# JulHoltzDevelopers/WavesAndEigenvalues.jl

Measured on AMD Instinct MI355X. Metric: eigenpairs/sec, higher is better.
Workload: dtype f64

## Files before the change

### wavesandeigenvalues.jl_amd/csrc/debug.hip

```cpp
#include <algorithm>
#include <vector>

#include "solver.h"

namespace {
struct StreamGuard {
    hipStream_t s = nullptr;
    ~StreamGuard() { if (s) (void)hipStreamDestroy(s); }
};
int64_t span(int64_t nv, int64_t stride, int64_t blk) { return nv > 0 ? (nv - 1) * stride + blk : 0; }
void fill_xorshift(std::vector<cplx> &hx) {
    uint64_t s = 0x9E3779B97F4A7C15ull;
    for (auto &v : hx) { s ^= s << 13; s ^= s >> 7; s ^= s << 17; v.x = (double)(s & 0xFFFFF) / 524288.0 - 1.0; v.y = (double)((s >> 20) & 0xFFFFF) / 524288.0 - 1.0; }
}
template <class F> double mean_ms(hipStream_t st, int reps, F &&one) {
    for (int i = 0; i < 3; ++i) one();
    hipEvent_t e0, e1;
    HIP_CHECK(hipEventCreate(&e0));
    HIP_CHECK(hipEventCreate(&e1));
    HIP_CHECK(hipEventRecord(e0, st));
    for (int i = 0; i < reps; ++i) one();
    HIP_CHECK(hipEventRecord(e1, st));
    HIP_CHECK(hipEventSynchronize(e1));
    float ms = 0.f;
// ... 217 lines not shown
            } else if (kind == WAE_GMRES_PAIR) {
                const int64_t onorm = off + (2 * (j + 1) + 3) * N;
                for (int b = 0; b < 2 * nb; ++b) hinv[(size_t)e * 2 * nb + b] = inv2(hpool[onorm + b].x);
            }
        }
        HIP_CHECK(hipSetDevice(device));
        StreamGuard sg;
        HIP_CHECK(hipStreamCreate(&sg.s));
        hipStream_t st = sg.s;
        const size_t nR = (size_t)m * (m + 1) * nb, nrow = (size_t)m * nb;
        DevBuf<cplx> dpool, R, sn, g, vsq, Hraw, rescale, dinv, s_rescale, s_vsq;
        DevBuf<double> cs, sv, sub, hist, relres, bn, s_relres, s_sv;
        DevBuf<int> ints, s_int;
        DevBuf<unsigned char> cmask, ddone, s_cmask;
        const cplx *hc = (const cplx *)cstate;
        dpool.upload(hpool, (size_t)plen, st);
        R.upload(hc, nR, st); sn.upload(hc + nR, nrow, st); g.upload(hc + nR + nrow, nrow + nb, st);
        vsq.upload(hc + nR + 2 * nrow + nb, nrow + 2 * nb, st); Hraw.upload(hc + nR + 3 * nrow + 3 * nb, nR, st);
        cs.upload(dstate, nrow, st); sv.upload(dstate + nrow, nrow + 2 * nb, st); sub.upload(dstate + 2 * nrow + 2 * nb, nrow, st);
        hist.upload(dstate + 3 * nrow + 2 * nb, (size_t)histcap * nb, st);
        bn.upload(bnorm, (size_t)nb, st);
        ddone.upload(hdone.data(), hdone.size(), st);
        dinv.upload(hinv.data(), hinv.size(), st);
        relres.alloc(nb); rescale.alloc(nb); ints.alloc(nint); cmask.alloc(nch);
        HIP_CHECK(hipMemsetAsync(ints.p, 0, (size_t)nint * sizeof(int), st));
        HIP_CHECK(hipMemsetAsync(relres.p, 0, (size_t)nb * sizeof(double), st));
        HIP_CHECK(hipMemsetAsync(rescale.p, 0, (size_t)nb * sizeof(cplx), st));
        HIP_CHECK(hipMemsetAsync(cmask.p, 0, (size_t)nch, st));
        s_relres.alloc((size_t)nev * nb); s_int.alloc((size_t)nev * nint); s_cmask.alloc((size_t)nev * nch); s_rescale.alloc((size_t)nev * nb);
        s_sv.alloc((size_t)nev * 2 * nb); s_vsq.alloc((size_t)nev * 2 * nb);
        HIP_CHECK(hipMemsetAsync(s_sv.p, 0, (size_t)nev * 2 * nb * sizeof(double), st));
        HIP_CHECK(hipMemsetAsync(s_vsq.p, 0, (size_t)nev * 2 * nb * sizeof(cplx), st));
        GmresDev S;
        S.nb = nb; S.m = m; S.histcap = histcap;
        S.R = R.p; S.cs = cs.p; S.sn = sn.p; S.g = g.p; S.sv = sv.p; S.vsq = vsq.p;
        S.conv = ints.p; S.steps = S.conv + nb; S.iters = S.steps + nb; S.histlen = S.iters + nb; S.stalled = S.histlen + nb; S.status = S.stalled + nb;
        S.relres = relres.p; S.bnorm = bn.p; S.hist = hist.p; S.rescale = rescale.p; S.cmask = cmask.p;
        S.Hraw = Hraw.p; S.sub = sub.p;
        auto d2d = [&](void *dst, const void *src, size_t bytes) { HIP_CHECK(hipMemcpyAsync(dst, src, bytes, hipMemcpyDeviceToDevice, st)); };
        for (int e = 0, ii = 0; e < nev; ++e) {
            const int64_t kind = ev[4 * e], j = ev[4 * e + 1], off = ev[4 * e + 3];
            const int use_mask = ev[4 * e + 2] ? 1 : 0;
            const double tol = evd[2 * e], lim = evd[2 * e + 1];
            cplx *a = dpool.p + off;
            int row0 = -1, rows = 0;
            if (kind == WAE_GMRES_INIT) {
                launch_gmres_init(S, a, ddone.p + (size_t)ii * nb, use_mask, st);
                ++ii;
                row0 = 0; rows = 1;
            } else if (kind == WAE_GMRES_STEP) {
                d2d(vsq.p + (size_t)(j + 1) * nb, dinv.p + (size_t)e * 2 * nb, (size_t)nb * sizeof(cplx));
                launch_gmres_step(S, a, (int)j, tol, lim, use_mask, a + (j + 2) * N, n, st);
                row0 = (int)j + 1; rows = 1;
            } else if (kind == WAE_GMRES_PAIR) {
                cplx *c1 = a, *c2 = c1 + (j + 1) * N, *gram = c2 + (j + 1) * N, *norms = gram + 3 * N, *W1 = norms + 2 * N, *W2 = W1 + blk,
                     *alpha = W2 + blk, *c2m = alpha + N, *hd2 = c2m + (j + 1) * N;
                launch_gmres_pair_coef(S, (int)j, c1, c2, gram, alpha, c2m, hd2, st);
                d2d(vsq.p + (size_t)(j + 1) * nb, dinv.p + (size_t)e * 2 * nb, (size_t)2 * nb * sizeof(cplx));
                launch_gmres_step(S, c1, (int)j, tol, 1e300, use_mask, W1, n, st, norms);
                launch_gmres_step(S, hd2, (int)j + 1, tol, lim, use_mask, W2, n, st, norms + N);
                row0 = (int)j + 1; rows = 2;
            } else {
                launch_gmres_solve_y(S, (int)j, a, st);
            }
            d2d(s_relres.p + (size_t)e * nb, relres.p, (size_t)nb * sizeof(double));
            d2d(s_int.p + (size_t)e * nint, ints.p, (size_t)nint * sizeof(int));
            d2d(s_cmask.p + (size_t)e * nch, cmask.p, (size_t)nch);
            d2d(s_rescale.p + (size_t)e * nb, rescale.p, (size_t)nb * sizeof(cplx));
            if (rows) {
                d2d(s_sv.p + (size_t)e * 2 * nb, sv.p + (size_t)row0 * nb, (size_t)rows * nb * sizeof(double));
                d2d(s_vsq.p + (size_t)e * 2 * nb, vsq.p + (size_t)row0 * nb, (size_t)rows * nb * sizeof(cplx));
            }
        }
        auto back = [&](void *dst, const void *src, size_t bytes) { HIP_CHECK(hipMemcpyAsync(dst, src, bytes, hipMemcpyDeviceToHost, st)); };
        cplx *oc = (cplx *)cstate;
        back(pool, dpool.p, (size_t)plen * sizeof(cplx));
        back(oc, R.p, nR * sizeof(cplx)); back(oc + nR, sn.p, nrow * sizeof(cplx)); back(oc + nR + nrow, g.p, (nrow + nb) * sizeof(cplx));
        back(oc + nR + 2 * nrow + nb, vsq.p, (nrow + 2 * nb) * sizeof(cplx)); back(oc + nR + 3 * nrow + 3 * nb, Hraw.p, nR * sizeof(cplx));
        back(dstate, cs.p, nrow * sizeof(double)); back(dstate + nrow, sv.p, (nrow + 2 * nb) * sizeof(double));
        back(dstate + 2 * nrow + 2 * nb, sub.p, nrow * sizeof(double)); back(dstate + 3 * nrow + 2 * nb, hist.p, (size_t)histcap * nb * sizeof(double));
        back(snap_relres, s_relres.p, (size_t)nev * nb * sizeof(double)); back(snap_int, s_int.p, (size_t)nev * nint * sizeof(int));
        back(snap_cmask, s_cmask.p, (size_t)nev * nch); back(snap_rescale, s_rescale.p, (size_t)nev * nb * sizeof(cplx));
        back(snap_sv, s_sv.p, (size_t)nev * 2 * nb * sizeof(double)); back(snap_vsq, s_vsq.p, (size_t)nev * 2 * nb * sizeof(cplx));
// ... 286 lines not shown
```

### wavesandeigenvalues.jl_amd/csrc/gmres.hip

```cpp
#include <cmath>

#include "solver.h"

void upload_pc(wae_family *h, const std::vector<std::vector<zc>> &pcs) {
    const int nsys = (int)pcs.size();
    const int nl = (int)h->ops.size();
    const size_t per_level = (size_t)nsys * h->nplanes;
    std::vector<cplx> tab(per_level * (nl + 2));
    for (int l = 0; l <= nl + 1; ++l) {
        if (l >= nl && h->n_penalty == 0) break;
        const std::vector<int> &sp = l < nl ? h->slot_plane[l] : (l == nl ? h->pen_slot : h->pen_row_slot);
        for (int s = 0; s < nsys; ++s) slot_coeffs(h, sp, pcs[s], &tab[l * per_level + (size_t)s * h->nplanes]);
    }
    h->pc_stride_level = per_level;
    h->pcdev.upload(tab.data(), tab.size(), h->stream);
    HIP_CHECK(hipStreamSynchronize(h->stream));
}
const cplx *pc_level(const wae_family *h, int l) { return h->pcdev.p + (size_t)l * h->pc_stride_level; }

void dense_setup(wae_family *h, const Batch &bt) {
    const int L = (int)h->ops.size() - 1;
    if (h->nc <= 0) return;
    HIP_CHECK(hipMemsetAsync(h->dstatus.p, 0, sizeof(int), h->stream));
    launch_dense_assemble(h->dense_planes.p, h->nplanes, (int)h->nc, pc_level(h, L), bt.nsys, bt.op, h->Ainv.p, h->stream);
// ... 245 lines not shown
                itot += iters[b];
                if (bnorm[b] > 0.0) {
                    if (!(relres[b] <= tol)) ++nun;
                    rmax = std::max(rmax, relres[b]);
                }
                if (stalled[b] && !(relres[b] <= tol)) info->levels |= 1 << 16;
            }
            info->iters_max = std::max(info->iters_max, imax);
            info->iters_total += itot;
            info->n_unconverged += nun;
            info->relres_max = std::max(info->relres_max, rmax);
            info->levels = (info->levels & (1 << 16)) | (int)h->ops.size();
        }
        if (nan_seen) throw WaeError(WAE_ERR_NAN, "NaN in GMRES");
        return total_it;
    }

    int run_device(wae_solve_info *info) {
        const GmresEnv &env = gmres_env();
        const double lim = env.lazy_limit;
        const bool use_mask = have_x0 || (env.mask0 && nb >= 8);
        const int nch = (nb + 7) / 8;
        const int histcap = maxit + m + 8;
        h->gs_R.reserve((size_t)m * (m + 1) * nb); h->gs_sn.reserve((size_t)m * nb); h->gs_g.reserve((size_t)(m + 1) * nb); h->gs_rescale.reserve((size_t)nb);
        h->gs_cs.reserve((size_t)m * nb); h->gs_sv.reserve((size_t)(m + 2) * nb); h->gs_relres.reserve((size_t)nb); h->gs_bnorm.reserve((size_t)nb);
        h->gs_hist.reserve((size_t)histcap * nb); h->gs_int.reserve((size_t)5 * nb + 4); h->gs_done.reserve((size_t)nb);
        h->cmask.reserve(nch); h->vsq.reserve((size_t)(m + 2) * nb);
        GmresDev S;
        S.nb = nb; S.m = m; S.histcap = histcap;
        S.R = h->gs_R.p; S.cs = h->gs_cs.p; S.sn = h->gs_sn.p; S.g = h->gs_g.p; S.sv = h->gs_sv.p; S.vsq = h->vsq.p;
        S.conv = h->gs_int.p; S.steps = S.conv + nb; S.iters = S.steps + nb; S.histlen = S.iters + nb; S.stalled = S.histlen + nb; S.status = S.stalled + nb;
        S.relres = h->gs_relres.p; S.bnorm = h->gs_bnorm.p; S.hist = h->gs_hist.p; S.rescale = h->gs_rescale.p; S.cmask = h->cmask.p;
        const int pair_min = env.pair_min;
        const bool pair_on = pair_min >= 0 && lim >= 1e50 && nb >= 8 && h->ops.size() > 1;
        h->gs_Hraw.reserve((size_t)m * (m + 1) * nb); h->gs_pair.reserve(((size_t)4 * (m + 3) + 8) * nb); h->gs_sub.reserve((size_t)m * nb);
        S.Hraw = h->gs_Hraw.p; S.sub = h->gs_sub.p;
        cplx *const pr_c1 = h->gs_pair.p, *const pr_c2 = pr_c1 + (size_t)(m + 3) * nb, *const pr_c2m = pr_c2 + (size_t)(m + 3) * nb,
                   *const pr_hd2 = pr_c2m + (size_t)(m + 3) * nb, *const pr_gram = pr_hd2 + (size_t)(m + 3) * nb, *const pr_alpha = pr_gram + (size_t)3 * nb,
                   *const pr_norm = pr_alpha + nb;
        HIP_CHECK(hipMemsetAsync(h->gs_int.p, 0, ((size_t)5 * nb + 4) * sizeof(int), st));
        cplx *const zb = start();
        std::vector<double> bn(bnorm);
        for (double &v : bn) if (!(v > 0.0)) v = 1.0;
        HIP_CHECK(hipMemcpyAsync(h->gs_bnorm.p, bn.data(), nb * sizeof(double), hipMemcpyHostToDevice, st));
        HIP_CHECK(hipStreamSynchronize(st));
        std::vector<int> hostint((size_t)5 * nb + 4);
        bool first = !have_x0;
// ... 8 lines not shown
            if (cycle_start([](int) {}) || total_it >= maxit || nan_seen) break;
            launch_scale_inv(z0, h->hdev.p, h->V.p, n, nb, st);
            HIP_CHECK(hipMemcpyAsync(h->gs_done.p, done.data(), nb, hipMemcpyHostToDevice, st));
            launch_gmres_init(S, h->hdev.p, h->gs_done.p, use_mask ? 1 : 0, st);
            HIP_CHECK(hipStreamSynchronize(st));
            const unsigned char *mk = (use_mask && nb >= 8) ? h->cmask.p : nullptr;
            int j = 0;
            int status[4] = {0, 0, 0, 0};
            for (int b = 0; b < nb; ++b) status[0] += done[b] ? 0 : 1;
            int since_sync = 0;
            for (; j < m && total_it < maxit;) {
                const cplx *vj = h->V.p + (size_t)j * vec;
                const int nvj = j + 1;
                const bool fuse0 = h->ops.size() > 1;
                if (pair_on && j >= pair_min && j + 2 <= m && total_it + 2 <= maxit && status[0] > nb / 4) {
                    cplx *w1 = h->V.p + (size_t)nvj * vec, *w2 = w1 + vec;
                    launch_spmv(A, pc, bt.cps, vj, h->W.p, h->lx[0].p, pre_weight(h), nb, MODE_AX_J0, st, mk);
                    vcycle(h, bt, 0, h->W.p, mk, true, w1);
                    launch_spmv(A, pc, bt.cps, w1, h->W.p, h->lx[0].p, pre_weight(h), nb, MODE_AX_J0, st, mk);
                    vcycle(h, bt, 0, h->W.p, mk, true, w2);
                    launch_dots2_scaled(h->V.p, vec, nvj, w1, w2, n, nb, h->partial.p, pr_c1, pr_c2, pr_gram, h->vsq.p, st, mk);
                    launch_gmres_pair_coef(S, j, pr_c1, pr_c2, pr_gram, pr_alpha, pr_c2m, pr_hd2, st);
                    launch_axpy2_norm(h->V.p, vec, nvj, pr_c1, pr_c2m, pr_alpha, w1, w2, n, nb, h->partial.p, pr_norm, h->vsq.p + (size_t)nvj * nb, st, mk);
                    launch_gmres_step(S, pr_c1, j, tol, 1e300, use_mask ? 1 : 0, w1, n, st, pr_norm);
                    launch_gmres_step(S, pr_hd2, j + 1, tol, lim, use_mask ? 1 : 0, w2, n, st, pr_norm + nb);
                    j += 2;
                    total_it += 2;
                    since_sync += 2;
                } else {
                    launch_spmv(A, pc, bt.cps, vj, h->W.p, fuse0 ? h->lx[0].p : nullptr, fuse0 ? pre_weight(h) : 0.0, nb, fuse0 ? MODE_AX_J0 : MODE_AX, st, mk);
                    cplx *w = vcycle(h, bt, 0, h->W.p, mk, fuse0);
                    launch_dots_scaled(h->V.p, vec, nvj, w, n, nb, h->partial.p, h->hdev.p, h->vsq.p, st, mk);
                    launch_axpy_neg_norm(h->V.p, vec, nvj, h->hdev.p, h->V.p + (size_t)nvj * vec, n, nb, h->partial.p, h->hdev.p + (size_t)nvj * nb, st, mk,
                                         w, h->vsq.p + (size_t)nvj * nb);
                    launch_gmres_step(S, h->hdev.p, j, tol, lim, use_mask ? 1 : 0, h->V.p + (size_t)nvj * vec, n, st);
                    ++j;
                    ++total_it;
                    ++since_sync;
                }
                if (since_sync >= ((have_x0 && j <= 4) ? 1 : env.sync) || j == m || total_it >= maxit || status[0] <= nb / 4) {
                    since_sync = 0;
                    HIP_CHECK(hipMemcpyAsync(status, S.status, 3 * sizeof(int), hipMemcpyDeviceToHost, st));
                    HIP_CHECK(hipStreamSynchronize(st));
                    if (status[1]) nan_seen = true;
                    if (status[0] == 0 || nan_seen) break;
                }
            }
            if (j > 0) {
// ... 434 lines not shown
```

### wavesandeigenvalues.jl_amd/csrc/vec.hip

```cpp
#include <type_traits>

#include "block_reduce.h"
#include "kernel_helpers.h"

__global__ void fill_zero_kernel(cplx *X, size_t count) {
    for (size_t e = (size_t)blockIdx.x * 256 + threadIdx.x; e < count; e += (size_t)gridDim.x * 256) X[e] = cplx{0.0, 0.0};
}
void launch_fill_zero(cplx *X, size_t count, hipStream_t st) {
    if (!count) return;
    hipLaunchKernelGGL(fill_zero_kernel, dim3(grid_for(count)), dim3(256), 0, st, X, count);
    HIP_CHECK(hipGetLastError());
}
void launch_copy(const cplx *X, cplx *Y, size_t count, hipStream_t st) {
    if (!count) return;
    HIP_CHECK(hipMemcpyAsync(Y, X, count * sizeof(cplx), hipMemcpyDeviceToDevice, st));
}
__global__ void add_kernel(const cplx *__restrict__ X, cplx *__restrict__ Y, size_t count) {
    for (size_t e = (size_t)blockIdx.x * 256 + threadIdx.x; e < count; e += (size_t)gridDim.x * 256) {
        cplx a = X[e], b = Y[e];
        Y[e] = cplx{a.x + b.x, a.y + b.y};
    }
}
void launch_add(const cplx *X, cplx *Y, size_t count, hipStream_t st) {
    if (!count) return;
// ... 742 lines not shown

__global__ __launch_bounds__(256) void gmres_init_kernel(GmresDev S, const cplx *__restrict__ beta, const unsigned char *__restrict__ done, int use_mask) {
    __shared__ int act[256];
    const int b = threadIdx.x;
    int a = 0;
    if (b < S.nb) {
        S.g[b] = cplx{beta[b].x, 0.0};
        S.sv[b] = 1.0;
        S.vsq[b] = cplx{1.0, 0.0};
        S.conv[b] = done[b] ? 1 : 0;
        S.steps[b] = 0;
        a = done[b] ? 0 : 1;
    }
    act[b] = a;
    __syncthreads();
    if (b < (S.nb + 7) / 8) {
        int any = 0;
        for (int k = 0; k < 8; ++k) any |= act[b * 8 + k];
        S.cmask[b] = use_mask ? (unsigned char)any : (unsigned char)1;
    }
    if (b == 0) {
        int n = 0;
        for (int k = 0; k < S.nb; ++k) n += act[k];
        S.status[0] = n; S.status[1] = 0; S.status[2] = 0;
    }
}

__global__ __launch_bounds__(256) void gmres_step_kernel(GmresDev S, const cplx *__restrict__ hd, int j, double tol, double lim, int use_mask,
                                                         const cplx *__restrict__ rn) {
    __shared__ int act[256];
    const int b = threadIdx.x;
    const int nb = S.nb, m = S.m;
    int a = 0;
    if (b < nb) {
        const int nvj = j + 1;
        const double sj = S.sv[(size_t)j * nb + b];
        const double r = rn ? rn[b].x : hd[(size_t)nvj * nb + b].x;
        if (S.Hraw) {
            cplx *Hr = S.Hraw + (size_t)j * (m + 1) * nb;
            for (int i = 0; i <= j; ++i) Hr[(size_t)i * nb + b] = hd[(size_t)i * nb + b];
        }
        double svn = r > 0.0 ? 1.0 / r : 0.0;
        const bool resc = svn > lim || (svn > 0.0 && svn < 1.0 / lim);
        S.rescale[b] = resc ? cplx{r, 0.0} : cplx{0.0, 0.0};
        if (S.sub) S.sub[(size_t)j * nb + b] = resc ? r : 1.0;
        if (resc) {
            S.vsq[(size_t)nvj * nb + b] = cplx{svn > 0.0 ? 1.0 : 0.0, 0.0};
            svn = svn > 0.0 ? 1.0 : 0.0;
            atomicOr(&S.status[2], 1);
        }
        S.sv[(size_t)nvj * nb + b] = svn;
        if (!S.conv[b]) {
            cplx *Hc = S.R + (size_t)j * (m + 1) * nb;
            for (int i = 0; i <= j; ++i) {
                const double si = S.sv[(size_t)i * nb + b];
                const double f = si > 0.0 ? sj / si : 0.0;
                const cplx c = hd[(size_t)i * nb + b];
                Hc[(size_t)i * nb + b] = cplx{c.x * f, c.y * f};
            }
            Hc[(size_t)(j + 1) * nb + b] = cplx{sj * r, 0.0};
            for (int i = 0; i < j; ++i) {
                const cplx aa = Hc[(size_t)i * nb + b], bb = Hc[(size_t)(i + 1) * nb + b];
                const double c = S.cs[(size_t)i * nb + b];
                const cplx sn = S.sn[(size_t)i * nb + b];
                const cplx sb = cmul(sn, bb), ca = cmul(cconj(sn), aa);
                Hc[(size_t)i * nb + b] = cplx{c * aa.x + sb.x, c * aa.y + sb.y};
                Hc[(size_t)(i + 1) * nb + b] = cplx{-ca.x + c * bb.x, -ca.y + c * bb.y};
            }
            const cplx av = Hc[(size_t)j * nb + b];
            const double bv = Hc[(size_t)(j + 1) * nb + b].x;
            const double aabs = hypot(av.x, av.y);
            const double t = sqrt(aabs * aabs + bv * bv);
            if (!(t > 0.0) || isnan(t)) {
                S.conv[b] = 1;
                if (isnan(t)) atomicOr(&S.status[1], 1);
            } else {
                double c;
                cplx sn;
                if (aabs == 0.0) { c = 0.0; sn = cplx{1.0, 0.0}; }
                else { c = aabs / t; const double q = bv / t; sn = cplx{av.x / aabs * q, av.y / aabs * q}; }
                S.cs[(size_t)j * nb + b] = c;
                S.sn[(size_t)j * nb + b] = sn;
                Hc[(size_t)j * nb + b] = cplx{c * av.x + sn.x * bv, c * av.y + sn.y * bv};
                Hc[(size_t)(j + 1) * nb + b] = cplx{0.0, 0.0};
                const cplx gj = S.g[(size_t)j * nb + b];
                const cplx gn = cmul(cconj(sn), gj);
                S.g[(size_t)(j + 1) * nb + b] = cplx{-gn.x, -gn.y};
                S.g[(size_t)j * nb + b] = cplx{c * gj.x, c * gj.y};
                S.steps[b] = j + 1;
                S.iters[b] += 1;
                const double rr = hypot(gn.x, gn.y) / S.bnorm[b];
                S.relres[b] = rr;
                if (isnan(rr)) atomicOr(&S.status[1], 1);
                const int hs = S.histlen[b];
                if (hs < S.histcap) { S.hist[(size_t)hs * nb + b] = rr; S.histlen[b] = hs + 1; }
                const int hn = hs + 1;
                if (rr <= 0.7 * tol) S.conv[b] = 1;
                else if (hn > 60 && hs < S.histcap && rr > 0.9 * S.hist[(size_t)(hn - 31) * nb + b]) { S.conv[b] = 1; S.stalled[b] = 1; }
                else a = 1;
            }
        }
    }
    act[b] = a;
    __syncthreads();
    if (b < (nb + 7) / 8 && use_mask) {
        int any = 0;
        for (int k = 0; k < 8; ++k) any |= act[b * 8 + k];
        S.cmask[b] = (unsigned char)any;
    }
    if (b == 0) {
        int n = 0;
        for (int k = 0; k < nb; ++k) n += act[k];
        S.status[0] = n;
    }
}

__global__ __launch_bounds__(256) void gmres_solve_y_kernel(GmresDev S, int ju, cplx *__restrict__ out) {
    const int b = threadIdx.x;
    const int nb = S.nb, m = S.m;
    if (b >= nb) return;
    const int k = S.steps[b];
    for (int i = k; i < ju; ++i) out[(size_t)i * nb + b] = cplx{0.0, 0.0};
    for (int i = k - 1; i >= 0; --i) {
        cplx sacc = S.g[(size_t)i * nb + b];
        for (int q = i + 1; q < k; ++q) {
            const cplx hq = S.R[((size_t)q * (m + 1) + i) * nb + b];
            const cplx yq = out[(size_t)q * nb + b];
            sacc.x -= hq.x * yq.x - hq.y * yq.y;
            sacc.y -= hq.x * yq.y + hq.y * yq.x;
        }
        const cplx dg = S.R[((size_t)i * (m + 1) + i) * nb + b];
        out[(size_t)i * nb + b] = (dg.x != 0.0 || dg.y != 0.0) ? cdiv(sacc, dg) : cplx{0.0, 0.0};
    }
    for (int i = 0; i < k; ++i) {
        const double f = S.sv[(size_t)i * nb + b];
        cplx y = out[(size_t)i * nb + b];
        out[(size_t)i * nb + b] = cplx{f * y.x, f * y.y};
    }
}

__global__ __launch_bounds__(256) void gmres_rescale_kernel(cplx *__restrict__ V, const cplx *__restrict__ factor, const int *__restrict__ status, size_t total, int nb) {
    if (!status[2]) return;
    for (size_t e = (size_t)blockIdx.x * 256 + threadIdx.x; e < total; e += (size_t)gridDim.x * 256) {
        const double f = factor[e % nb].x;
        if (f > 0.0) { const cplx x = V[e]; V[e] = cplx{x.x / f, x.y / f}; }
    }
}
__global__ void gmres_clear_rescale_kernel(int *status) { status[2] = 0; }

void launch_gmres_init(const GmresDev &S, const cplx *beta, const unsigned char *done, int use_mask, hipStream_t st) {
    hipLaunchKernelGGL(gmres_init_kernel, dim3(1), dim3(256), 0, st, S, beta, done, use_mask);
    HIP_CHECK(hipGetLastError());
}
__global__ __launch_bounds__(256) void gmres_pair_coef_kernel(GmresDev S, int j, const cplx *__restrict__ c1, const cplx *__restrict__ c2,
                                                              const cplx *__restrict__ gram, cplx *__restrict__ alpha, cplx *__restrict__ c2m,
                                                              cplx *__restrict__ hd2) {
    const int b = threadIdx.x;
    const int nb = S.nb, m = S.m;
    if (b >= nb) return;
    double uu = gram[b].x;
    cplx u12 = gram[(size_t)nb + b];
    for (int i = 0; i <= j; ++i) {
        const double q = S.vsq[(size_t)i * nb + b].x;
        const double w = q > 0.0 ? 1.0 / q : 0.0;
        const cplx a = c1[(size_t)i * nb + b], c = c2[(size_t)i * nb + b];
        uu -= (a.x * a.x + a.y * a.y) * w;
        u12.x -= (a.x * c.x + a.y * c.y) * w;
        u12.y -= (a.x * c.y - a.y * c.x) * w;
    }
    cplx al = {0.0, 0.0};
    if (uu > 0.0 && uu > 1e-28 * gram[b].x) al = cplx{u12.x / uu, u12.y / uu};
// ... 1 lines not shown
    cplx *Hj = S.Hraw + (size_t)j * (m + 1) * nb;
    for (int i = 0; i <= j; ++i) {
        const cplx a = c1[(size_t)i * nb + b], c = c2[(size_t)i * nb + b];
        Hj[(size_t)i * nb + b] = a;
        c2m[(size_t)i * nb + b] = cplx{c.x - (al.x * a.x - al.y * a.y), c.y - (al.x * a.y + al.y * a.x)};
    }
    S.sub[(size_t)j * nb + b] = 1.0;
    for (int i = 0; i <= j + 1; ++i) {
        cplx t = i <= j ? c2[(size_t)i * nb + b] : al;
        for (int k = i; k <= j; ++k) {
            const cplx hk = S.Hraw[((size_t)k * (m + 1) + i) * nb + b], ck = c1[(size_t)k * nb + b];
            t.x -= hk.x * ck.x - hk.y * ck.y;
            t.y -= hk.x * ck.y + hk.y * ck.x;
        }
        if (i >= 1) {
            const double sb = S.sub[(size_t)(i - 1) * nb + b];
            const cplx ck = c1[(size_t)(i - 1) * nb + b];
            t.x -= sb * ck.x;
            t.y -= sb * ck.y;
        }
        hd2[(size_t)i * nb + b] = t;
    }
}
void launch_gmres_pair_coef(const GmresDev &S, int j, const cplx *c1, const cplx *c2, const cplx *gram, cplx *alpha, cplx *c2m, cplx *hd2, hipStream_t st) {
    hipLaunchKernelGGL(gmres_pair_coef_kernel, dim3(1), dim3(256), 0, st, S, j, c1, c2, gram, alpha, c2m, hd2);
    HIP_CHECK(hipGetLastError());
}
void launch_gmres_step(const GmresDev &S, const cplx *hd, int j, double tol, double lim, int use_mask, cplx *Vnew, int64_t n, hipStream_t st,
                       const cplx *rn) {
    hipLaunchKernelGGL(gmres_step_kernel, dim3(1), dim3(256), 0, st, S, hd, j, tol, lim, use_mask, rn);
    hipLaunchKernelGGL(gmres_rescale_kernel, dim3(512), dim3(256), 0, st, Vnew, S.rescale, S.status, (size_t)n * S.nb, S.nb);
    hipLaunchKernelGGL(gmres_clear_rescale_kernel, dim3(1), dim3(1), 0, st, S.status);
    HIP_CHECK(hipGetLastError());
}
void launch_gmres_solve_y(const GmresDev &S, int ju, cplx *out, hipStream_t st) {
    hipLaunchKernelGGL(gmres_solve_y_kernel, dim3(1), dim3(256), 0, st, S, ju, out);
    HIP_CHECK(hipGetLastError());
}

__global__ __launch_bounds__(256) void triad_kernel(double2 *__restrict__ a, const double2 *__restrict__ b, const double2 *__restrict__ c, double s, size_t n2) {
    for (size_t e = (size_t)blockIdx.x * 256 + threadIdx.x; e < n2; e += (size_t)gridDim.x * 256) {
        double2 x = b[e], y = c[e];
        a[e] = double2{x.x + s * y.x, x.y + s * y.y};
    }
}
void launch_triad(double *a, const double *b, const double *c, double s_, int64_t n, hipStream_t st, unsigned grid_cap) {
    size_t n2 = (size_t)n / 2;
    hipLaunchKernelGGL(triad_kernel, dim3(grid_for(n2, grid_cap)), dim3(256), 0, st, (double2 *)a, (const double2 *)b, (const double2 *)c, s_, n2);
    HIP_CHECK(hipGetLastError());
}

constexpr int PTG_MAXW = 3072;
template <int TMAX>
__global__ __launch_bounds__(256) void pt_gemm_batch_kernel(const cplx *__restrict__ V, size_t stride, int k, const cplx *__restrict__ G, int T, int t0,
                                                            int tn, cplx *__restrict__ U, int64_t d, int nb, int accumulate) {
    extern __shared__ cplx ptg_w[];
    const int tid = threadIdx.x;
    for (int e = tid; e < k * tn * nb; e += 256) {
        const int b = e % nb, it = e / nb, t = it % tn, i = it / tn;
// ... 104 lines not shown
```

### wavesandeigenvalues.jl_amd/csrc/wae_internal.h

```cpp
#pragma once
#include <hip/hip_runtime.h>
#include <algorithm>
#include <cmath>
#include <complex>
#include <cstdint>
#include <cstdio>
#include <cstring>
#include <stdexcept>
#include <string>
#include <vector>

#include "../../include/waehip.h"

typedef std::complex<double> zc;
typedef double2 cplx;

struct WaeError : std::runtime_error {
    int code;
    WaeError(int c, const std::string &m) : std::runtime_error(m), code(c) {}
};
void wae_set_error(const std::string &m);
int wae_internal_device(const wae_family *h);
hipStream_t wae_internal_stream(const wae_family *h);

// ... 291 lines not shown
    cplx *R;
    double *cs;
    cplx *sn;
    cplx *g;
    double *sv;
    cplx *vsq;
    int *conv, *steps, *iters, *histlen, *stalled;
    double *relres, *bnorm;
    double *hist;
    cplx *rescale;
    int *status;
    unsigned char *cmask;
    cplx *Hraw;
    double *sub;
};
void launch_gmres_init(const GmresDev &S, const cplx *beta, const unsigned char *done, int use_mask, hipStream_t s);
void launch_gmres_step(const GmresDev &S, const cplx *hd, int j, double tol, double lim, int use_mask, cplx *Vnew, int64_t n, hipStream_t s,
                       const cplx *rn = nullptr);
void launch_dots2_scaled(const cplx *V, size_t stride, int nv, const cplx *W1, const cplx *W2, int64_t n, int nb, cplx *partial, cplx *out1,
                         cplx *out2, cplx *gram_out, const cplx *scale, hipStream_t s, const unsigned char *cmask = nullptr);
void launch_axpy2_norm(const cplx *V, size_t stride, int nv, const cplx *c1, const cplx *c2m, const cplx *alpha, cplx *W1, cplx *W2, int64_t n, int nb,
                       cplx *partial, cplx *norms, cplx *inv_out, hipStream_t s, const unsigned char *cmask = nullptr);
void launch_gmres_pair_coef(const GmresDev &S, int j, const cplx *c1, const cplx *c2, const cplx *gram, cplx *alpha, cplx *c2m, cplx *hd2, hipStream_t s);
void launch_gmres_solve_y(const GmresDev &S, int ju, cplx *out, hipStream_t s);
void launch_forced_rhs(const int *rows, const cplx *M, int64_t nr, int nsrc, const cplx *G, cplx *B, int nb, hipStream_t s);
void launch_forced_observe(const int64_t *ptr, const int *idx, const cplx *val, int nobs, const cplx *X, int nb, cplx *H, int64_t j0, hipStream_t s);
void launch_triad(double *a, const double *b, const double *c, double s, int64_t n, hipStream_t st, unsigned grid_cap = 8192);
```

Measured before the change: 4.433.

## Fuse paired GMRES steps into one LDS-staged kernel and parallelize small solves

Paired Arnoldi columns now go through a single step kernel that applies both Givens updates in one launch. The Hessenberg column and Givens coefficients are staged in shared memory, the rescale kernel handles both vectors together, and the clear-rescale launch is dropped. The pair-coefficient and triangular-solve kernels gain LDS-backed multi-block variants that spread the work across more workgroups instead of one block. This targets launch overhead and serial global-memory latency in these small single-block kernels. In exchange it adds LDS-size fallbacks, a larger rescale buffer and new status-slot semantics that must stay consistent.

```diff
diff --git a/wavesandeigenvalues.jl_amd/csrc/debug.hip b/wavesandeigenvalues.jl_amd/csrc/debug.hip
--- a/wavesandeigenvalues.jl_amd/csrc/debug.hip
+++ b/wavesandeigenvalues.jl_amd/csrc/debug.hip
@@ -263,10 +263,10 @@
         bn.upload(bnorm, (size_t)nb, st);
         ddone.upload(hdone.data(), hdone.size(), st);
         dinv.upload(hinv.data(), hinv.size(), st);
-        relres.alloc(nb); rescale.alloc(nb); ints.alloc(nint); cmask.alloc(nch);
+        relres.alloc(nb); rescale.alloc((size_t)2 * nb); ints.alloc(nint); cmask.alloc(nch);
         HIP_CHECK(hipMemsetAsync(ints.p, 0, (size_t)nint * sizeof(int), st));
         HIP_CHECK(hipMemsetAsync(relres.p, 0, (size_t)nb * sizeof(double), st));
-        HIP_CHECK(hipMemsetAsync(rescale.p, 0, (size_t)nb * sizeof(cplx), st));
+        HIP_CHECK(hipMemsetAsync(rescale.p, 0, (size_t)2 * nb * sizeof(cplx), st));
         HIP_CHECK(hipMemsetAsync(cmask.p, 0, (size_t)nch, st));
         s_relres.alloc((size_t)nev * nb); s_int.alloc((size_t)nev * nint); s_cmask.alloc((size_t)nev * nch); s_rescale.alloc((size_t)nev * nb);
         s_sv.alloc((size_t)nev * 2 * nb); s_vsq.alloc((size_t)nev * 2 * nb);
@@ -298,8 +298,7 @@
                      *alpha = W2 + blk, *c2m = alpha + N, *hd2 = c2m + (j + 1) * N;
                 launch_gmres_pair_coef(S, (int)j, c1, c2, gram, alpha, c2m, hd2, st);
                 d2d(vsq.p + (size_t)(j + 1) * nb, dinv.p + (size_t)e * 2 * nb, (size_t)2 * nb * sizeof(cplx));
-                launch_gmres_step(S, c1, (int)j, tol, 1e300, use_mask, W1, n, st, norms);
-                launch_gmres_step(S, hd2, (int)j + 1, tol, lim, use_mask, W2, n, st, norms + N);
+                launch_gmres_pair_step(S, c1, hd2, (int)j, tol, 1e300, lim, use_mask, W1, W2, n, st, norms);
                 row0 = (int)j + 1; rows = 2;
             } else {
                 launch_gmres_solve_y(S, (int)j, a, st);
diff --git a/wavesandeigenvalues.jl_amd/csrc/gmres.hip b/wavesandeigenvalues.jl_amd/csrc/gmres.hip
--- a/wavesandeigenvalues.jl_amd/csrc/gmres.hip
+++ b/wavesandeigenvalues.jl_amd/csrc/gmres.hip
@@ -291,7 +291,7 @@
         const bool use_mask = have_x0 || (env.mask0 && nb >= 8);
         const int nch = (nb + 7) / 8;
         const int histcap = maxit + m + 8;
-        h->gs_R.reserve((size_t)m * (m + 1) * nb); h->gs_sn.reserve((size_t)m * nb); h->gs_g.reserve((size_t)(m + 1) * nb); h->gs_rescale.reserve((size_t)nb);
+        h->gs_R.reserve((size_t)m * (m + 1) * nb); h->gs_sn.reserve((size_t)m * nb); h->gs_g.reserve((size_t)(m + 1) * nb); h->gs_rescale.reserve((size_t)2 * nb);
         h->gs_cs.reserve((size_t)m * nb); h->gs_sv.reserve((size_t)(m + 2) * nb); h->gs_relres.reserve((size_t)nb); h->gs_bnorm.reserve((size_t)nb);
         h->gs_hist.reserve((size_t)histcap * nb); h->gs_int.reserve((size_t)5 * nb + 4); h->gs_done.reserve((size_t)nb);
         h->cmask.reserve(nch); h->vsq.reserve((size_t)(m + 2) * nb);
@@ -346,8 +346,7 @@
                     launch_dots2_scaled(h->V.p, vec, nvj, w1, w2, n, nb, h->partial.p, pr_c1, pr_c2, pr_gram, h->vsq.p, st, mk);
                     launch_gmres_pair_coef(S, j, pr_c1, pr_c2, pr_gram, pr_alpha, pr_c2m, pr_hd2, st);
                     launch_axpy2_norm(h->V.p, vec, nvj, pr_c1, pr_c2m, pr_alpha, w1, w2, n, nb, h->partial.p, pr_norm, h->vsq.p + (size_t)nvj * nb, st, mk);
-                    launch_gmres_step(S, pr_c1, j, tol, 1e300, use_mask ? 1 : 0, w1, n, st, pr_norm);
-                    launch_gmres_step(S, pr_hd2, j + 1, tol, lim, use_mask ? 1 : 0, w2, n, st, pr_norm + nb);
+                    launch_gmres_pair_step(S, pr_c1, pr_hd2, j, tol, 1e300, lim, use_mask ? 1 : 0, w1, w2, n, st, pr_norm);
                     j += 2;
                     total_it += 2;
                     since_sync += 2;
diff --git a/wavesandeigenvalues.jl_amd/csrc/vec.hip b/wavesandeigenvalues.jl_amd/csrc/vec.hip
--- a/wavesandeigenvalues.jl_amd/csrc/vec.hip
+++ b/wavesandeigenvalues.jl_amd/csrc/vec.hip
@@ -788,103 +788,188 @@
     if (b == 0) {
         int n = 0;
         for (int k = 0; k < S.nb; ++k) n += act[k];
-        S.status[0] = n; S.status[1] = 0; S.status[2] = 0;
-    }
-}
-
-__global__ __launch_bounds__(256) void gmres_step_kernel(GmresDev S, const cplx *__restrict__ hd, int j, double tol, double lim, int use_mask,
-                                                         const cplx *__restrict__ rn) {
+        S.status[0] = n; S.status[1] = 0; S.status[2] = 0; S.status[3] = 0;
+    }
+}
+
+constexpr size_t GMRES_LDS_BUDGET = 144 * 1024;
+static void gmres_lds_opt_in(const void *kernel) { HIP_CHECK(hipFuncSetAttribute(kernel, hipFuncAttributeMaxDynamicSharedMemorySize, (int)GMRES_LDS_BUDGET)); }
+
+struct GmresColumn { int conv, iters, hs; double bnorm; cplx g; };
+
+__device__ __forceinline__ void gmres_stage_column(const GmresDev &S, const cplx *__restrict__ hd, int j, const double *sjl, cplx *Hc) {
+    const int nb = S.nb, total = (j + 1) * nb;
+    cplx *Hr = S.Hraw ? S.Hraw + (size_t)j * (S.m + 1) * nb : nullptr;
+    for (int e0 = threadIdx.x; e0 < total; e0 += 4 * 256) {
+        cplx c[4];
+        double si[4];
+#pragma unroll
+        for (int u = 0; u < 4; ++u) {
+            const int e = e0 + u * 256;
+            c[u] = cplx{0.0, 0.0}; si[u] = 0.0;
+            if (e < total) { c[u] = hd[e]; si[u] = S.sv[e]; }
+        }
+#pragma unroll
+        for (int u = 0; u < 4; ++u) {
+            const int e = e0 + u * 256;
+            if (e < total) {
+                const int i = e / nb, b = e - i * nb;
+                const double sj = sjl[b], s = i == j ? sj : si[u];
+                const double f = s > 0.0 ? sj / s : 0.0;
+                if (Hr) Hr[e] = c[u];
+                Hc[e] = cplx{c[u].x * f, c[u].y * f};
+            }
+        }
+    }
+}
+
+__device__ __forceinline__ int gmres_step_column(const GmresDev &S, const cplx *__restrict__ hd, int j, double tol, double lim, const cplx *__restrict__ rn,
+                                                 int b, bool staged, bool keep, cplx *Hc, double *csl, cplx *snl, double sj, cplx *resc_out,
+                                                 GmresColumn &col, int &resc_any, double &svn_out) {
+    const int nb = S.nb, m = S.m, nvj = j + 1;
+    const double r = rn ? rn[b].x : hd[(size_t)nvj * nb + b].x;
+    if (!staged && S.Hraw) {
+        cplx *Hr = S.Hraw + (size_t)j * (m + 1) * nb;
+        for (int i = 0; i <= j; ++i) Hr[(size_t)i * nb + b] = hd[(size_t)i * nb + b];
+    }
+    double svn = r > 0.0 ? 1.0 / r : 0.0;
+    const bool resc = svn > lim || (svn > 0.0 && svn < 1.0 / lim);
+    resc_out[b] = resc ? cplx{r, 0.0} : cplx{0.0, 0.0};
+    if (S.sub) S.sub[(size_t)j * nb + b] = resc ? r : 1.0;
+    if (resc) {
+        S.vsq[(size_t)nvj * nb + b] = cplx{svn > 0.0 ? 1.0 : 0.0, 0.0};
+        svn = svn > 0.0 ? 1.0 : 0.0;
+        resc_any = 1;
+    }
+    S.sv[(size_t)nvj * nb + b] = svn;
+    svn_out = svn;
+    if (col.conv) return 0;
+    if (!staged) {
+        for (int i = 0; i <= j; ++i) {
+            const double si = S.sv[(size_t)i * nb + b];
+            const double f = si > 0.0 ? sj / si : 0.0;
+            const cplx c = hd[(size_t)i * nb + b];
+            Hc[(size_t)i * nb + b] = cplx{c.x * f, c.y * f};
+        }
+    }
+    const double bv = sj * r;
+    cplx aa = Hc[b];
+    for (int i = 0; i < j; ++i) {
+        const cplx bb = Hc[(size_t)(i + 1) * nb + b];
+        const double c = csl[(size_t)i * nb + b];
+        const cplx sn = snl[(size_t)i * nb + b];
+        const cplx sb = cmul(sn, bb), ca = cmul(cconj(sn), aa);
+        Hc[(size_t)i * nb + b] = cplx{c * aa.x + sb.x, c * aa.y + sb.y};
+        aa = cplx{-ca.x + c * bb.x, -ca.y + c * bb.y};
+    }
+    const cplx av = aa;
+    const double aabs = hypot(av.x, av.y);
+    const double t = sqrt(aabs * aabs + bv * bv);
+    int a = 0;
+    if (!(t > 0.0) || isnan(t)) {
+        Hc[(size_t)j * nb + b] = av;
+        Hc[(size_t)(j + 1) * nb + b] = cplx{bv, 0.0};
+        col.conv = 1;
+        S.conv[b] = 1;
+        if (isnan(t)) atomicOr(&S.status[1], 1);
+    } else {
+        double c;
+        cplx sn;
+        if (aabs == 0.0) { c = 0.0; sn = cplx{1.0, 0.0}; }
+        else { c = aabs / t; const double q = bv / t; sn = cplx{av.x / aabs * q, av.y / aabs * q}; }
+        S.cs[(size_t)j * nb + b] = c;
+        S.sn[(size_t)j * nb + b] = sn;
+        if (keep) { csl[(size_t)j * nb + b] = c; snl[(size_t)j * nb + b] = sn; }
+        Hc[(size_t)j * nb + b] = cplx{c * av.x + sn.x * bv, c * av.y + sn.y * bv};
+        Hc[(size_t)(j + 1) * nb + b] = cplx{0.0, 0.0};
+        const cplx gj = col.g;
+        const cplx gn = cmul(cconj(sn), gj);
+        col.g = cplx{-gn.x, -gn.y};
+        S.g[(size_t)(j + 1) * nb + b] = col.g;
+        S.g[(size_t)j * nb + b] = cplx{c * gj.x, c * gj.y};
+        S.steps[b] = j + 1;
+        col.iters += 1;
+        S.iters[b] = col.iters;
+        const double rr = hypot(gn.x, gn.y) / col.bnorm;
+        S.relres[b] = rr;
+        if (isnan(rr)) atomicOr(&S.status[1], 1);
+        const int hs = col.hs;
+        if (hs < S.histcap) { S.hist[(size_t)hs * nb + b] = rr; col.hs = hs + 1; S.histlen[b] = hs + 1; }
+        const int hn = hs + 1;
+        if (rr <= 0.7 * tol) { col.conv = 1; S.conv[b] = 1; }
+        else if (hn > 60 && hs < S.histcap && rr > 0.9 * S.hist[(size_t)(hn - 31) * nb + b]) { col.conv = 1; S.conv[b] = 1; S.stalled[b] = 1; }
+        else a = 1;
+    }
+    if (staged) {
+        cplx *Rc = S.R + (size_t)j * (m + 1) * nb;
+        for (int i = 0; i <= j + 1; ++i) Rc[(size_t)i * nb + b] = Hc[(size_t)i * nb + b];
+    }
+    return a;
+}
+
+__global__ __launch_bounds__(256) void gmres_step_kernel(GmresDev S, const cplx *__restrict__ hd1, const cplx *__restrict__ hd2, int j, double tol,
+                                                         double lim1, double lim2, int use_mask, const cplx *__restrict__ rn, int staged) {
+    extern __shared__ cplx step_lds[];
     __shared__ int act[256];
+    __shared__ double sjl[256];
     const int b = threadIdx.x;
     const int nb = S.nb, m = S.m;
-    int a = 0;
+    const int jmax = hd2 ? j + 1 : j;
+    cplx *Hl = step_lds, *snl = Hl + (size_t)(jmax + 2) * nb;
+    double *csl = (double *)(snl + (size_t)jmax * nb);
+    GmresColumn col = {1, 0, 0, 1.0, cplx{0.0, 0.0}};
     if (b < nb) {
-        const int nvj = j + 1;
-        const double sj = S.sv[(size_t)j * nb + b];
-        const double r = rn ? rn[b].x : hd[(size_t)nvj * nb + b].x;
-        if (S.Hraw) {
-            cplx *Hr = S.Hraw + (size_t)j * (m + 1) * nb;
-            for (int i = 0; i <= j; ++i) Hr[(size_t)i * nb + b] = hd[(size_t)i * nb + b];
-        }
-        double svn = r > 0.0 ? 1.0 / r : 0.0;
-        const bool resc = svn > lim || (svn > 0.0 && svn < 1.0 / lim);
-        S.rescale[b] = resc ? cplx{r, 0.0} : cplx{0.0, 0.0};
-        if (S.sub) S.sub[(size_t)j * nb + b] = resc ? r : 1.0;
-        if (resc) {
-            S.vsq[(size_t)nvj * nb + b] = cplx{svn > 0.0 ? 1.0 : 0.0, 0.0};
-            svn = svn > 0.0 ? 1.0 : 0.0;
-            atomicOr(&S.status[2], 1);
-        }
-        S.sv[(size_t)nvj * nb + b] = svn;
-        if (!S.conv[b]) {
-            cplx *Hc = S.R + (size_t)j * (m + 1) * nb;
-            for (int i = 0; i <= j; ++i) {
-                const double si = S.sv[(size_t)i * nb + b];
-                const double f = si > 0.0 ? sj / si : 0.0;
-                const cplx c = hd[(size_t)i * nb + b];
-                Hc[(size_t)i * nb + b] = cplx{c.x * f, c.y * f};
-            }
-            Hc[(size_t)(j + 1) * nb + b] = cplx{sj * r, 0.0};
-            for (int i = 0; i < j; ++i) {
-                const cplx aa = Hc[(size_t)i * nb + b], bb = Hc[(size_t)(i + 1) * nb + b];
-                const double c = S.cs[(size_t)i * nb + b];
-                const cplx sn = S.sn[(size_t)i * nb + b];
-                const cplx sb = cmul(sn, bb), ca = cmul(cconj(sn), aa);
-                Hc[(size_t)i * nb + b] = cplx{c * aa.x + sb.x, c * aa.y + sb.y};
-                Hc[(size_t)(i + 1) * nb + b] = cplx{-ca.x + c * bb.x, -ca.y + c * bb.y};
-            }
-            const cplx av = Hc[(size_t)j * nb + b];
-            const double bv = Hc[(size_t)(j + 1) * nb + b].x;
-            const double aabs = hypot(av.x, av.y);
-            const double t = sqrt(aabs * aabs + bv * bv);
-            if (!(t > 0.0) || isnan(t)) {
-                S.conv[b] = 1;
-                if (isnan(t)) atomicOr(&S.status[1], 1);
-            } else {
-                double c;
-                cplx sn;
-                if (aabs == 0.0) { c = 0.0; sn = cplx{1.0, 0.0}; }
-                else { c = aabs / t; const double q = bv / t; sn = cplx{av.x / aabs * q, av.y / aabs * q}; }
-                S.cs[(size_t)j * nb + b] = c;
-                S.sn[(size_t)j * nb + b] = sn;
-                Hc[(size_t)j * nb + b] = cplx{c * av.x + sn.x * bv, c * av.y + sn.y * bv};
-                Hc[(size_t)(j + 1) * nb + b] = cplx{0.0, 0.0};
-                const cplx gj = S.g[(size_t)j * nb + b];
-                const cplx gn = cmul(cconj(sn), gj);
-                S.g[(size_t)(j + 1) * nb + b] = cplx{-gn.x, -gn.y};
-                S.g[(size_t)j * nb + b] = cplx{c * gj.x, c * gj.y};
-                S.steps[b] = j + 1;
-                S.iters[b] += 1;
-                const double rr = hypot(gn.x, gn.y) / S.bnorm[b];
-                S.relres[b] = rr;
-                if (isnan(rr)) atomicOr(&S.status[1], 1);
-                const int hs = S.histlen[b];
-                if (hs < S.histcap) { S.hist[(size_t)hs * nb + b] = rr; S.histlen[b] = hs + 1; }
-                const int hn = hs + 1;
-                if (rr <= 0.7 * tol) S.conv[b] = 1;
-                else if (hn > 60 && hs < S.histcap && rr > 0.9 * S.hist[(size_t)(hn - 31) * nb + b]) { S.conv[b] = 1; S.stalled[b] = 1; }
-                else a = 1;
-            }
-        }
+        col = GmresColumn{S.conv[b], S.iters[b], S.histlen[b], S.bnorm[b], S.g[(size_t)j * nb + b]};
+        sjl[b] = S.sv[(size_t)j * nb + b];
+    }
+    if (staged) {
+        const int total = j * nb;
+        for (int e0 = b; e0 < total; e0 += 4 * 256) {
+            cplx s[4];
+            double c[4];
+#pragma unroll
+            for (int u = 0; u < 4; ++u) {
+                const int e = e0 + u * 256;
+                s[u] = cplx{0.0, 0.0}; c[u] = 0.0;
+                if (e < total) { s[u] = S.sn[e]; c[u] = S.cs[e]; }
+            }
+#pragma unroll
+            for (int u = 0; u < 4; ++u) {
+                const int e = e0 + u * 256;
+                if (e < total) { snl[e] = s[u]; csl[e] = c[u]; }
+            }
+        }
+    }
+    __syncthreads();
+    if (staged) gmres_stage_column(S, hd1, j, sjl, Hl);
+    __syncthreads();
+    int a = 0, resc_any = 0;
+    double svn = 0.0;
+    if (b < nb)
+        a = gmres_step_column(S, hd1, j, tol, lim1, rn, b, staged, staged && hd2, staged ? Hl : S.R + (size_t)j * (m + 1) * nb, staged ? csl : S.cs,
+                              staged ? snl : S.sn, sjl[b], hd2 ? S.rescale + nb : S.rescale, col, resc_any, svn);
+    if (hd2) {
+        if (b < nb) sjl[b] = svn;
+        __syncthreads();
+        if (staged) gmres_stage_column(S, hd2, j + 1, sjl, Hl);
+        __syncthreads();
+        if (b < nb)
+            a = gmres_step_column(S, hd2, j + 1, tol, lim2, rn + nb, b, staged, false, staged ? Hl : S.R + (size_t)(j + 1) * (m + 1) * nb,
+                                  staged ? csl : S.cs, staged ? snl : S.sn, svn, S.rescale, col, resc_any, svn);
     }
     act[b] = a;
-    __syncthreads();
+    const int nact = __syncthreads_count(a);
+    const int anyr = __syncthreads_or(resc_any);
     if (b < (nb + 7) / 8 && use_mask) {
         int any = 0;
         for (int k = 0; k < 8; ++k) any |= act[b * 8 + k];
         S.cmask[b] = (unsigned char)any;
     }
-    if (b == 0) {
-        int n = 0;
-        for (int k = 0; k < nb; ++k) n += act[k];
-        S.status[0] = n;
-    }
-}
-
-__global__ __launch_bounds__(256) void gmres_solve_y_kernel(GmresDev S, int ju, cplx *__restrict__ out) {
-    const int b = threadIdx.x;
+    if (b == 0) { S.status[0] = nact; S.status[3] = anyr ? 1 : 0; }
+}
+
+__device__ __forceinline__ void gmres_solve_y_column(const GmresDev &S, int ju, cplx *__restrict__ out, int b) {
     const int nb = S.nb, m = S.m;
-    if (b >= nb) return;
     const int k = S.steps[b];
     for (int i = k; i < ju; ++i) out[(size_t)i * nb + b] = cplx{0.0, 0.0};
     for (int i = k - 1; i >= 0; --i) {
@@ -904,15 +989,85 @@
         out[(size_t)i * nb + b] = cplx{f * y.x, f * y.y};
     }
 }
-
-__global__ __launch_bounds__(256) void gmres_rescale_kernel(cplx *__restrict__ V, const cplx *__restrict__ factor, const int *__restrict__ status, size_t total, int nb) {
-    if (!status[2]) return;
+__global__ __launch_bounds__(256) void gmres_solve_y_kernel(GmresDev S, int ju, cplx *__restrict__ out) {
+    if ((int)threadIdx.x < S.nb) gmres_solve_y_column(S, ju, out, threadIdx.x);
+}
+__global__ __launch_bounds__(256) void gmres_solve_y_lds_kernel(GmresDev S, int ju, cplx *__restrict__ out, int cpw) {
+    extern __shared__ cplx solve_lds[];
+    __shared__ int ks[256];
+    const int tid = threadIdx.x;
+    const int nb = S.nb, m = S.m;
+    const int b0 = blockIdx.x * cpw;
+    const int nc = min(cpw, nb - b0);
+    const int T = ju * (ju + 1) / 2;
+    cplx *tri = solve_lds, *gl = tri + (size_t)T * cpw, *yl = gl + (size_t)ju * cpw;
+    if (tid < nc) ks[tid] = S.steps[b0 + tid];
+    __syncthreads();
+    const int total = ju * ju * nc;
+    for (int e0 = tid; e0 < total; e0 += 8 * 256) {
+        cplx v[8];
+        int at[8];
+#pragma unroll
+        for (int u = 0; u < 8; ++u) {
+            const int e = e0 + u * 256;
+            at[u] = -1;
+            v[u] = cplx{0.0, 0.0};
+            if (e < total) {
+                const int c = e % nc, r = e / nc, q = r / ju, i = r - q * ju;
+                if (i <= q && q < ks[c]) {
+                    at[u] = (q * (q + 1) / 2 + i) * cpw + c;
+                    v[u] = S.R[((size_t)q * (m + 1) + i) * nb + b0 + c];
+                }
+            }
+        }
+#pragma unroll
+        for (int u = 0; u < 8; ++u)
+            if (at[u] >= 0) tri[at[u]] = v[u];
+    }
+    for (int e = tid; e < ju * nc; e += 256) {
+        const int c = e % nc, i = e / nc;
+        if (i < ks[c]) gl[i * cpw + c] = S.g[(size_t)i * nb + b0 + c];
+    }
+    __syncthreads();
+    if (tid < nc) {
+        const int c = tid, k = ks[c];
+        if (k > ju) gmres_solve_y_column(S, ju, out, b0 + c);
+        else {
+            for (int i = k - 1; i >= 0; --i) {
+                cplx sacc = gl[i * cpw + c];
+                for (int q = i + 1; q < k; ++q) {
+                    const cplx hq = tri[(q * (q + 1) / 2 + i) * cpw + c];
+                    const cplx yq = yl[q * cpw + c];
+                    sacc.x -= hq.x * yq.x - hq.y * yq.y;
+                    sacc.y -= hq.x * yq.y + hq.y * yq.x;
+                }
+                const cplx dg = tri[(i * (i + 1) / 2 + i) * cpw + c];
+                yl[i * cpw + c] = (dg.x != 0.0 || dg.y != 0.0) ? cdiv(sacc, dg) : cplx{0.0, 0.0};
+            }
+        }
+    }
+    __syncthreads();
+    for (int e = tid; e < ju * nc; e += 256) {
+        const int c = e % nc, i = e / nc, k = ks[c];
+        if (k > ju) continue;
+        cplx y = {0.0, 0.0};
+        if (i < k) { const double f = S.sv[(size_t)i * nb + b0 + c]; const cplx t = yl[i * cpw + c]; y = cplx{f * t.x, f * t.y}; }
+        out[(size_t)i * nb + b0 + c] = y;
+    }
+}
+
+__global__ __launch_bounds__(256) void gmres_rescale_kernel(cplx *__restrict__ V1, cplx *__restrict__ V2, const cplx *__restrict__ factor,
+                                                            const int *__restrict__ status, size_t total, int nb) {
+    if (!status[3]) return;
     for (size_t e = (size_t)blockIdx.x * 256 + threadIdx.x; e < total; e += (size_t)gridDim.x * 256) {
         const double f = factor[e % nb].x;
-        if (f > 0.0) { const cplx x = V[e]; V[e] = cplx{x.x / f, x.y / f}; }
-    }
-}
-__global__ void gmres_clear_rescale_kernel(int *status) { status[2] = 0; }
+        if (f > 0.0) { const cplx x = V2[e]; V2[e] = cplx{x.x / f, x.y / f}; }
+        if (V1) {
+            const double f1 = factor[nb + e % nb].x;
+            if (f1 > 0.0) { const cplx x = V1[e]; V1[e] = cplx{x.x / f1, x.y / f1}; }
+        }
+    }
+}
 
 void launch_gmres_init(const GmresDev &S, const cplx *beta, const unsigned char *done, int use_mask, hipStream_t st) {
     hipLaunchKernelGGL(gmres_init_kernel, dim3(1), dim3(256), 0, st, S, beta, done, use_mask);
@@ -960,19 +1115,126 @@
         hd2[(size_t)i * nb + b] = t;
     }
 }
+__global__ __launch_bounds__(256) void gmres_pair_coef_lds_kernel(GmresDev S, int j, const cplx *__restrict__ c1, const cplx *__restrict__ c2,
+                                                                  const cplx *__restrict__ gram, cplx *__restrict__ alpha, cplx *__restrict__ c2m,
+                                                                  cplx *__restrict__ hd2, int rpb) {
+    extern __shared__ cplx coef_lds[];
+    __shared__ cplx all[256];
+    const int tid = threadIdx.x;
+    const int nb = S.nb, m = S.m;
+    const int total = (j + 1) * nb;
+    cplx *c1l = coef_lds, *c2l = c1l + total;
+    double *wl = (double *)(c2l + total);
+    for (int e0 = tid; e0 < total; e0 += 4 * 256) {
+        cplx a[4], c[4];
+        double q[4];
+#pragma unroll
+        for (int u = 0; u < 4; ++u) {
+            const int e = e0 + u * 256;
+            a[u] = c[u] = cplx{0.0, 0.0}; q[u] = 0.0;
+            if (e < total) { a[u] = c1[e]; c[u] = c2[e]; q[u] = S.vsq[e].x; }
+        }
+#pragma unroll
+        for (int u = 0; u < 4; ++u) {
+            const int e = e0 + u * 256;
+            if (e < total) { c1l[e] = a[u]; c2l[e] = c[u]; wl[e] = q[u] > 0.0 ? 1.0 / q[u] : 0.0; }
+        }
+    }
+    __syncthreads();
+    if (tid < nb) {
+        const int b = tid;
+        double uu = gram[b].x;
+        cplx u12 = gram[(size_t)nb + b];
+        for (int i = 0; i <= j; ++i) {
+            const double w = wl[i * nb + b];
+            const cplx a = c1l[i * nb + b], c = c2l[i * nb + b];
+            uu -= (a.x * a.x + a.y * a.y) * w;
+            u12.x -= (a.x * c.x + a.y * c.y) * w;
+            u12.y -= (a.x * c.y - a.y * c.x) * w;
+        }
+        cplx al = {0.0, 0.0};
+        if (uu > 0.0 && uu > 1e-28 * gram[b].x) al = cplx{u12.x / uu, u12.y / uu};
+        all[b] = al;
+        if (blockIdx.x == 0) { alpha[b] = al; S.sub[(size_t)j * nb + b] = 1.0; }
+    }
+    __syncthreads();
+    const int il = tid / nb, b = tid - il * nb;
+    const int i = blockIdx.x * rpb + il;
+    if (il >= rpb || i > j + 1) return;
+    const cplx al = all[b];
+    if (i <= j) {
+        const cplx a = c1l[i * nb + b], c = c2l[i * nb + b];
+        S.Hraw[((size_t)j * (m + 1) + i) * nb + b] = a;
+        c2m[(size_t)i * nb + b] = cplx{c.x - (al.x * a.x - al.y * a.y), c.y - (al.x * a.y + al.y * a.x)};
+    }
+    cplx t = i <= j ? c2l[i * nb + b] : al;
+    int k = i;
+    for (; k + 8 <= j; k += 8) {
+        cplx h[8];
+#pragma unroll
+        for (int u = 0; u < 8; ++u) h[u] = S.Hraw[((size_t)(k + u) * (m + 1) + i) * nb + b];
+#pragma unroll
+        for (int u = 0; u < 8; ++u) {
+            const cplx hk = h[u], ck = c1l[(k + u) * nb + b];
+            t.x -= hk.x * ck.x - hk.y * ck.y;
+            t.y -= hk.x * ck.y + hk.y * ck.x;
+        }
+    }
+    for (; k <= j; ++k) {
+        const cplx hk = k < j ? S.Hraw[((size_t)k * (m + 1) + i) * nb + b] : c1l[i * nb + b], ck = c1l[k * nb + b];
+        t.x -= hk.x * ck.x - hk.y * ck.y;
+        t.y -= hk.x * ck.y + hk.y * ck.x;
+    }
+    if (i >= 1) {
+        const double sb = i - 1 < j ? S.sub[(size_t)(i - 1) * nb + b] : 1.0;
+        const cplx ck = c1l[(i - 1) * nb + b];
+        t.x -= sb * ck.x;
+        t.y -= sb * ck.y;
+    }
+    hd2[(size_t)i * nb + b] = t;
+}
 void launch_gmres_pair_coef(const GmresDev &S, int j, const cplx *c1, const cplx *c2, const cplx *gram, cplx *alpha, cplx *c2m, cplx *hd2, hipStream_t st) {
-    hipLaunchKernelGGL(gmres_pair_coef_kernel, dim3(1), dim3(256), 0, st, S, j, c1, c2, gram, alpha, c2m, hd2);
+    const size_t shm = (size_t)(j + 1) * S.nb * (2 * sizeof(cplx) + sizeof(double));
+    if (shm <= GMRES_LDS_BUDGET) {
+        static OncePerDevice lds_opt_in;
+        once_per_device(lds_opt_in, [](int) { gmres_lds_opt_in((const void *)gmres_pair_coef_lds_kernel); });
+        const int rpb = std::max(1, 256 / S.nb);
+        hipLaunchKernelGGL(gmres_pair_coef_lds_kernel, dim3((j + 2 + rpb - 1) / rpb), dim3(256), shm, st, S, j, c1, c2, gram, alpha, c2m, hd2, rpb);
+    } else {
+        hipLaunchKernelGGL(gmres_pair_coef_kernel, dim3(1), dim3(256), 0, st, S, j, c1, c2, gram, alpha, c2m, hd2);
+    }
+    HIP_CHECK(hipGetLastError());
+}
+static void gmres_steps(const GmresDev &S, const cplx *hd1, const cplx *hd2, int j, double tol, double lim1, double lim2, int use_mask, cplx *V1, cplx *V2,
+                        int64_t n, hipStream_t st, const cplx *rn) {
+    const int jmax = hd2 ? j + 1 : j;
+    const size_t shm = (size_t)S.nb * ((size_t)(jmax + 2) * sizeof(cplx) + (size_t)jmax * (sizeof(cplx) + sizeof(double)));
+    const int staged = shm <= GMRES_LDS_BUDGET ? 1 : 0;
+    static OncePerDevice lds_opt_in;
+    once_per_device(lds_opt_in, [](int) { gmres_lds_opt_in((const void *)gmres_step_kernel); });
+    hipLaunchKernelGGL(gmres_step_kernel, dim3(1), dim3(256), staged ? shm : 0, st, S, hd1, hd2, j, tol, lim1, lim2, use_mask, rn, staged);
+    hipLaunchKernelGGL(gmres_rescale_kernel, dim3(512), dim3(256), 0, st, V1, V2, S.rescale, S.status, (size_t)n * S.nb, S.nb);
     HIP_CHECK(hipGetLastError());
 }
 void launch_gmres_step(const GmresDev &S, const cplx *hd, int j, double tol, double lim, int use_mask, cplx *Vnew, int64_t n, hipStream_t st,
                        const cplx *rn) {
-    hipLaunchKernelGGL(gmres_step_kernel, dim3(1), dim3(256), 0, st, S, hd, j, tol, lim, use_mask, rn);
-    hipLaunchKernelGGL(gmres_rescale_kernel, dim3(512), dim3(256), 0, st, Vnew, S.rescale, S.status, (size_t)n * S.nb, S.nb);
-    hipLaunchKernelGGL(gmres_clear_rescale_kernel, dim3(1), dim3(1), 0, st, S.status);
-    HIP_CHECK(hipGetLastError());
+    gmres_steps(S, hd, nullptr, j, tol, lim, lim, use_mask, nullptr, Vnew, n, st, rn);
+}
+void launch_gmres_pair_step(const GmresDev &S, const cplx *hd1, const cplx *hd2, int j, double tol, double lim1, double lim2, int use_mask, cplx *W1,
+                            cplx *W2, int64_t n, hipStream_t st, const cplx *norms) {
+    if (!hd2 || !norms) throw WaeError(WAE_ERR_INVALID, "gmres_pair_step: the second column and the two norms are required");
+    gmres_steps(S, hd1, hd2, j, tol, lim1, lim2, use_mask, W1, W2, n, st, norms);
 }
 void launch_gmres_solve_y(const GmresDev &S, int ju, cplx *out, hipStream_t st) {
-    hipLaunchKernelGGL(gmres_solve_y_kernel, dim3(1), dim3(256), 0, st, S, ju, out);
+    const size_t percol = ((size_t)ju * (ju + 1) / 2 + 2 * (size_t)ju) * sizeof(cplx);
+    const int cpw = (int)std::min<size_t>(std::min(S.nb, 16), GMRES_LDS_BUDGET / percol);
+    if (cpw >= 1) {
+        static OncePerDevice lds_opt_in;
+        once_per_device(lds_opt_in, [](int) { gmres_lds_opt_in((const void *)gmres_solve_y_lds_kernel); });
+        hipLaunchKernelGGL(gmres_solve_y_lds_kernel, dim3((S.nb + cpw - 1) / cpw), dim3(256), percol * cpw, st, S, ju, out, cpw);
+    } else {
+        hipLaunchKernelGGL(gmres_solve_y_kernel, dim3(1), dim3(256), 0, st, S, ju, out);
+    }
     HIP_CHECK(hipGetLastError());
 }
 
diff --git a/wavesandeigenvalues.jl_amd/csrc/wae_internal.h b/wavesandeigenvalues.jl_amd/csrc/wae_internal.h
--- a/wavesandeigenvalues.jl_amd/csrc/wae_internal.h
+++ b/wavesandeigenvalues.jl_amd/csrc/wae_internal.h
@@ -337,6 +337,8 @@
 void launch_axpy2_norm(const cplx *V, size_t stride, int nv, const cplx *c1, const cplx *c2m, const cplx *alpha, cplx *W1, cplx *W2, int64_t n, int nb,
                        cplx *partial, cplx *norms, cplx *inv_out, hipStream_t s, const unsigned char *cmask = nullptr);
 void launch_gmres_pair_coef(const GmresDev &S, int j, const cplx *c1, const cplx *c2, const cplx *gram, cplx *alpha, cplx *c2m, cplx *hd2, hipStream_t s);
+void launch_gmres_pair_step(const GmresDev &S, const cplx *hd1, const cplx *hd2, int j, double tol, double lim1, double lim2, int use_mask, cplx *W1,
+                            cplx *W2, int64_t n, hipStream_t s, const cplx *norms);
 void launch_gmres_solve_y(const GmresDev &S, int ju, cplx *out, hipStream_t s);
 void launch_forced_rhs(const int *rows, const cplx *M, int64_t nr, int nsrc, const cplx *G, cplx *B, int nb, hipStream_t s);
 void launch_forced_observe(const int64_t *ptr, const int *idx, const cplx *val, int nobs, const cplx *X, int nb, cplx *H, int64_t j0, hipStream_t s);
```

After: 4.407. Within noise of the previous version (-0.6%).
